# tum-pbs/DMCF

Hardware: AMD Instinct MI355X
Metric: rollout_particle_steps_per_sec (higher is better)
Workload: dtype f32

## Files before the change

dmcf_amd/csrc/cconv_cls.hip:

```cpp

#include "cconv_common.h"

namespace dmcf {

constexpr int kCWaves = 8;
constexpr int kCThreads = 64 * kCWaves;
constexpr int CTM = 2 * kCWaves;
constexpr int kCRows = 16;
constexpr int CCH = 16;
constexpr int kCRow = 1024;
constexpr int kSlots = 96;
constexpr int kHalfSlots = 48;
constexpr int kGrp = 20;
constexpr int kXst = 512;
constexpr int kCMaxNT = 4;
constexpr int kNoPair = 9;

#define CLS_TILE_REGS                                                                                                     \
    "v92", "v93", "v94", "v95", "v96", "v97", "v98", "v99", "v100", "v101", "v102", "v103", "v104", "v105", "v106", "v107", \
        "v108", "v109", "v110", "v111", "v112", "v113", "v114", "v115", "v116", "v117", "v118", "v119", "v120", "v121",    \
        "v122", "v123", "v124", "v125", "v126", "v127"
constexpr int kClsCompilerVgprs = 46;

__device__ __forceinline__ void cls_zero_tiles() {
    asm volatile(
        "v_mov_b32 v92, 0\n\tv_mov_b32 v93, 0\n\tv_mov_b32 v94, 0\n\tv_mov_b32 v95, 0\n\t"
        "v_mov_b32 v96, 0\n\tv_mov_b32 v97, 0\n\tv_mov_b32 v98, 0\n\tv_mov_b32 v99, 0\n\t"
        "v_mov_b32 v100, 0\n\tv_mov_b32 v101, 0\n\tv_mov_b32 v102, 0\n\tv_mov_b32 v103, 0\n\t"
        "v_mov_b32 v104, 0\n\tv_mov_b32 v105, 0\n\tv_mov_b32 v106, 0\n\tv_mov_b32 v107, 0\n\t"
        "v_mov_b32 v108, 0\n\tv_mov_b32 v109, 0\n\tv_mov_b32 v110, 0\n\tv_mov_b32 v111, 0\n\t"
        "v_mov_b32 v112, 0\n\tv_mov_b32 v113, 0\n\tv_mov_b32 v114, 0\n\tv_mov_b32 v115, 0\n\t"
        "v_mov_b32 v116, 0\n\tv_mov_b32 v117, 0\n\tv_mov_b32 v118, 0\n\tv_mov_b32 v119, 0\n\t"
        "v_mov_b32 v120, 0\n\tv_mov_b32 v121, 0\n\tv_mov_b32 v122, 0\n\tv_mov_b32 v123, 0\n\t"
        "v_mov_b32 v124, 0\n\tv_mov_b32 v125, 0\n\tv_mov_b32 v126, 0\n\tv_mov_b32 v127, 0"
        ::: "memory", CLS_TILE_REGS);
}

struct ClsRec {
    float x;
    f32x4 w;
};

__device__ __forceinline__ uint32_t cls_lds_addr(const void* q) {
    return (uint32_t)(uintptr_t)(const __attribute__((address_space(3))) void*)q;
}

__device__ __forceinline__ void xfence() {
    __builtin_amdgcn_fence(__ATOMIC_RELEASE, "wavefront");
    __builtin_amdgcn_wave_barrier();
    __builtin_amdgcn_fence(__ATOMIC_ACQUIRE, "wavefront");
}

template <int NTT, bool NARROW, bool SYM, bool SINGLE, bool PLAIN>
__global__ __launch_bounds__(kCThreads, 4) __attribute__((amdgpu_num_vgpr(kClsCompilerVgprs))) void cconv_cls_kernel(const CconvParams p) {
    extern __shared__ __attribute__((aligned(16))) float smem[];
    const int tid = threadIdx.x, lane = tid & 63;
    const int wave = __builtin_amdgcn_readfirstlane(tid >> 6);
    const int cin = p.cin, cout = p.cout;
    float* Bt = smem;
    float* Gs = smem + CTM * kCRow + wave * kXst;
    unsigned char* Cst = (unsigned char*)(Gs + 24 * kGrp);
    float* Fst = Bt + (wave + kCWaves) * kCRow;
    int* Jst = (int*)(Fst + kHalfSlots * 16);
    const int tile = (int)(blockIdx.x % 8) * p.tiles_per_xcd + (int)(blockIdx.x / 8);
    if (tile >= p.ntiles) return;
    const int64_t pt0 = (int64_t)tile * CTM;
    const int window = PLAIN ? (int)DMCF_WINDOW_POLY6 : p.window;
    const float* const nval = PLAIN ? nullptr : p.nval;
    const float* const imp = PLAIN ? nullptr : p.inp_imp;
    constexpr bool symmetric = SYM;

    const int mk = lane >> 4, mn = lane & 15;
    const float xm = (float)(lane & 3);
    const int widx = (lane >> 2) & 3;
    const int mi = lane & 15, mg = lane >> 4;
    const uint32_t gs_lds = cls_lds_addr(Gs), fst_lds = cls_lds_addr(Fst);
    constexpr uint32_t kOob = 0xffffffffu;
    const uint32_t rowB = (uint32_t)cin * 4u;
    const __amdgpu_buffer_rsrc_t rF = __builtin_amdgcn_make_buffer_rsrc((void*)p.inp_feat, 0, (int)((uint32_t)p.n_inp * rowB), 0x00020000);

    f32x4 acc[NTT];
#pragma unroll
    for (int n = 0; n < NTT; ++n) acc[n] = (f32x4){0.0f, 0.0f, 0.0f, 0.0f};

    float out_prev = 0.0f;
    for (int chunk = 0; chunk < p.nchunks; ++chunk) {
        const int c0 = chunk * CCH;
        const int nch = min(CCH, cin - c0);
        constexpr bool narrow = NARROW;
        const int fr = narrow ? lane >> 1 : lane >> 2, fc4 = narrow ? lane & 1 : lane & 3;
        const int spi = narrow ? 32 : 16;
        const int fstride = narrow ? 8 : 16;
        const bool fch_ok = c0 + 4 * fc4 < cin;
        const int fch = fch_ok ? c0 + 4 * fc4 : 0;
        int64_t rbs[2];
        int nts[2], nbs[2];
        float oxs[2], oys[2], ozs[2];
#pragma unroll
        for (int pp = 0; pp < 2; ++pp) {
            const int64_t i = pt0 + wave + kCWaves * pp;
            rbs[pp] = 0;
            nts[pp] = 0;
            oxs[pp] = oys[pp] = ozs[pp] = 0.0f;
            if (i < p.n_out) {
                const int64_t rb = p.rs[i];
                int64_t re = p.cnt ? rb + p.cnt[i] : p.rs[i + 1];
                if (re > p.pair_cap) re = rb;
                rbs[pp] = rb;
                nts[pp] = (int)min(re - rb, (int64_t)0x7fffffc0);
                oxs[pp] = p.out_pos[3 * i];
                oys[pp] = p.out_pos[3 * i + 1];
                ozs[pp] = p.out_pos[3 * i + 2];
            }
            nbs[pp] = (nts[pp] + 63) >> 6;
        }
        const int nbA = nbs[0], NB = nbs[0] + nbs[1];
        cls_zero_tiles();

        const int nt0 = __builtin_amdgcn_readfirstlane(nts[0]), nt1 = __builtin_amdgcn_readfirstlane(nts[1]);
        const int64_t rb0 = ((int64_t)__builtin_amdgcn_readfirstlane((int)(rbs[0] >> 32)) << 32) | (uint32_t)__builtin_amdgcn_readfirstlane((int)rbs[0]);
        const int64_t rb1 = ((int64_t)__builtin_amdgcn_readfirstlane((int)(rbs[1] >> 32)) << 32) | (uint32_t)__builtin_amdgcn_readfirstlane((int)rbs[1]);
        const int64_t gapB = nt1 > 0 ? rb1 - rb0 : 0;
        const bool near = gapB >= 0 && gapB + nt1 < ((int64_t)1 << 29) && nt0 < (1 << 29);
        const __amdgpu_buffer_rsrc_t rI = __builtin_amdgcn_make_buffer_rsrc(
            (void*)(p.idx + rb0), 0, near ? (int)(max((int64_t)nt0, gapB + nt1) * 4) : 0, 0x00020000);
        const uint32_t offB = (uint32_t)gapB * 4u;
        auto valid = [&](int t) -> bool {
            const bool pp = t >= nbA;
            return t < NB && 64 * (t - (pp ? nbA : 0)) + lane < (pp ? nt1 : nt0);
        };
        auto ld_idx = [&](int t, int& j, float& nv) {
            const bool pp = t >= nbA, ok = valid(t);
            const int o = 64 * (t - (pp ? nbA : 0)) + lane;
            j = 0;
            nv = 0.0f;
            if (near) {
                j = (int)__builtin_amdgcn_raw_buffer_load_b32(rI, ok ? (uint32_t)o * 4u + (pp ? offB : 0u) : kOob, 0, 0);
            } else if (ok) {
                j = p.idx[(pp ? rb1 : rb0) + o];
            }
            if (nval && ok) nv = nval[(pp ? rb1 : rb0) + o];
        };
        auto ld_pos = [&](int j, float& x, float& y, float& z) {
            const float* q = (const float*)((const char*)p.inp_pos + (size_t)__umul24((uint32_t)j, 12u));
            x = q[0];
            y = q[1];
            z = q[2];
        };
        auto geom = [&](int t, int j, float nv, float x, float y, float z, int& cls) -> ClsRec {
            ClsRec c;
            const bool pp = t >= nbA;
            x -= pp ? oxs[1] : oxs[0];
            y -= pp ? oys[1] : oys[0];
            z -= pp ? ozs[1] : ozs[0];
            float a = window_value(window, nval ? nv : rel_dist2(x, y, z), p.inv_r2, p.window_fac);
            if (imp) a *= imp[j];
            filter_coords<false>(x, y, z, p);
            c.x = fminf(3.0f, fmaxf(0.0f, x));
            y = fminf(3.0f, fmaxf(0.0f, y));
            z = fminf(3.0f, fmaxf(0.0f, z));
            const float yf = fminf(floorf(y), 2.0f), zf = fminf(floorf(z), 2.0f);
            const float fy = y - yf, fz = z - zf;
            cls = valid(t) ? 3 * (int)zf + (int)yf : kNoPair;
            const float a0 = a * (1.0f - fz), a1 = a * fz;
            c.w = (f32x4){a0 * (1.0f - fy), a0 * fy, a1 * (1.0f - fy), a1 * fy};
            return c;
        };
        struct Order {
            int pos;
            int cb[10];
        };
        auto order = [&](int cls) -> Order {
            Order o;
            o.pos = 0;
            int base = 0;
#pragma unroll
            for (int c = 0; c < 9; ++c) {
                const uint64_t m = __ballot(cls == c);
                const int rank = __builtin_amdgcn_mbcnt_hi((uint32_t)(m >> 32), __builtin_amdgcn_mbcnt_lo((uint32_t)m, base));
                o.pos = cls == c ? rank : o.pos;
                o.cb[c] = base;
                base += (__builtin_popcountll(m) + 3) & ~3;
            }
            o.cb[9] = base;
            return o;
        };
        auto push_index = [&](int j, int cls, int pos) {
            Jst[lane] = -1;
            if (lane < kSlots - 64) Jst[64 + lane] = -1;
            xfence();
            if (cls != kNoPair) Jst[pos] = (int)__umul24((uint32_t)j, rowB);
        };
        auto push_rec = [&](const ClsRec& c, int cls, int pos) {
            *(f32x4*)(Gs + 4 * lane) = (f32x4){0.0f, 0.0f, 0.0f, 0.0f};
            if (lane < kGrp * 6 - 64) *(f32x4*)(Gs + 4 * (64 + lane)) = (f32x4){0.0f, 0.0f, 0.0f, 0.0f};
            xfence();
            if (cls != kNoPair) {
                float* g = Gs + (pos >> 2) * kGrp + (pos & 3);
                g[16] = c.x;
                *(f32x4*)(g + 3 * (pos & 3)) = c.w;
                if ((pos & 3) == 0) Cst[pos >> 2] = (unsigned char)(4 * cls);
            }
        };
        const uint32_t cbyte = fch_ok ? 4u * (uint32_t)fch : kOob;
        auto f_issue = [&](int h, f32x4 (&f)[3]) {
            uint32_t jo[3];
#pragma unroll
            for (int k = 0; k < 3; ++k) jo[k] = (uint32_t)Jst[kHalfSlots * h + spi * k + fr];
#pragma unroll
            for (int k = 0; k < 3; ++k)
                f[k] = __builtin_bit_cast(f32x4, __builtin_amdgcn_raw_buffer_load_b128(rF, __builtin_elementwise_add_sat(jo[k], cbyte), 0, 0));
        };
        auto f_publish = [&](int t, const f32x4 (&f)[3]) {
            if constexpr (symmetric) {
                f32x4 fi4 = {0.0f, 0.0f, 0.0f, 0.0f};
                if (fch_ok) fi4 = *(const f32x4*)(p.inp_feat + (pt0 + wave + (t >= nbA ? kCWaves : 0)) * cin + fch);
#pragma unroll
                for (int k = 0; k < 3; ++k) *(f32x4*)(Fst + (spi * k + fr) * fstride + 4 * fc4) = f[k] + fi4;
            } else {
#pragma unroll
                for (int k = 0; k < 3; ++k) *(f32x4*)(Fst + (spi * k + fr) * fstride + 4 * fc4) = f[k];
            }
        };
        auto splat = [&](int h, int nslots) {
            const int lo = kHalfSlots * h;
            const int ng = (min(lo + kHalfSlots, nslots) - lo) >> 2;
            const uint32_t pw = gs_lds + ((lo >> 2) * kGrp + 4 * mk + widx) * 4;
            const uint32_t px = gs_lds + ((lo >> 2) * kGrp + 16 + mk) * 4;
            const uint32_t pf = fst_lds + (16 * mk + mn) * 4;
            const uint32_t* cw = (const uint32_t*)(Cst + (lo >> 2));
            const uint32_t c0 = __builtin_amdgcn_readfirstlane(cw[0]), c1 = __builtin_amdgcn_readfirstlane(cw[1]),
                           c2 = __builtin_amdgcn_readfirstlane(cw[2]);
            float xa, wa, fa, xb, wb, fb, av;
            uint32_t sc;
            __builtin_amdgcn_s_setprio(3);
            asm volatile(
#include "cconv_cls_splat.inc"
                : [xa] "=&v"(xa), [wa] "=&v"(wa), [fa] "=&v"(fa), [xb] "=&v"(xb), [wb] "=&v"(wb), [fb] "=&v"(fb),
                  [a] "=&v"(av), [sc] "=&s"(sc)
                : [px] "v"(px), [pw] "v"(pw), [pf] "v"(pf), [xm] "v"(xm), [ng] "s"(ng), [c0] "s"(c0), [c1] "s"(c1), [c2] "s"(c2)
                : "scc", "m0", "memory", CLS_TILE_REGS);
            __builtin_amdgcn_s_setprio(0);
        };
        auto splat8 = [&](int nslots) {
            const int ng = nslots >> 2;
            const uint32_t pw = gs_lds + (4 * mk + widx) * 4;
            const uint32_t px = gs_lds + (16 + mk) * 4;
            const uint32_t pf = fst_lds + (8 * mk + (mn & 7)) * 4;
            const uint32_t* cw = (const uint32_t*)Cst;
            uint32_t c[6];
#pragma unroll
            for (int q = 0; q < 6; ++q) c[q] = __builtin_amdgcn_readfirstlane(cw[q]);
            float xa, wa, fa, xb, wb, fb, av;
            uint32_t sc;
            __builtin_amdgcn_s_setprio(3);
            asm volatile(
#include "cconv_cls_splat8.inc"
                : [xa] "=&v"(xa), [wa] "=&v"(wa), [fa] "=&v"(fa), [xb] "=&v"(xb), [wb] "=&v"(wb), [fb] "=&v"(fb),
                  [a] "=&v"(av), [sc] "=&s"(sc)
                : [px] "v"(px), [pw] "v"(pw), [pf] "v"(pf), [xm] "v"(xm), [ng] "s"(ng), [c0] "s"(c[0]), [c1] "s"(c[1]),
                  [c2] "s"(c[2]), [c3] "s"(c[3]), [c4] "s"(c[4]), [c5] "s"(c[5])
                : "scc", "m0", "memory", CLS_TILE_REGS);
            __builtin_amdgcn_s_setprio(0);
        };
        auto merge = [&](int pt) {
            float* Brow = Bt + pt * kCRow;
            const int gz = lane >> 5, gy = (lane >> 4) & 1;
            const int col = (mn ^ (pt & 15)) << 2;
            const uint32_t mb = cls_lds_addr(Brow + (gz * 4 + gy) * 64 + col);
            xfence();
            asm volatile(
                "s_nop 7\n\ts_nop 7\n\ts_nop 7\n\t"
                "ds_write_b128 %[b], v[92:95] offset:0\n\t"
                "ds_write_b128 %[b], v[100:103] offset:512\n\t"
                "ds_write_b128 %[b], v[116:119] offset:2048\n\t"
                "ds_write_b128 %[b], v[124:127] offset:2560\n\t"
                "ds_read_b128 v[92:95], %[b] offset:256\n\t"
                "s_waitcnt lgkmcnt(0)\n\t"
                "v_add_f32 v92, v92, v96\n\tv_add_f32 v93, v93, v97\n\tv_add_f32 v94, v94, v98\n\tv_add_f32 v95, v95, v99\n\t"
                "ds_write_b128 %[b], v[92:95] offset:256\n\t"
                "ds_read_b128 v[92:95], %[b] offset:2304\n\t"
                "s_waitcnt lgkmcnt(0)\n\t"
                "v_add_f32 v92, v92, v120\n\tv_add_f32 v93, v93, v121\n\tv_add_f32 v94, v94, v122\n\tv_add_f32 v95, v95, v123\n\t"
                "ds_write_b128 %[b], v[92:95] offset:2304\n\t"
                "ds_read_b128 v[92:95], %[b] offset:1024\n\t"
                "s_waitcnt lgkmcnt(0)\n\t"
                "v_add_f32 v92, v92, v104\n\tv_add_f32 v93, v93, v105\n\tv_add_f32 v94, v94, v106\n\tv_add_f32 v95, v95, v107\n\t"
                "ds_write_b128 %[b], v[92:95] offset:1024\n\t"
                "ds_read_b128 v[92:95], %[b] offset:1536\n\t"
                "s_waitcnt lgkmcnt(0)\n\t"
                "v_add_f32 v92, v92, v112\n\tv_add_f32 v93, v93, v113\n\tv_add_f32 v94, v94, v114\n\tv_add_f32 v95, v95, v115\n\t"
                "ds_write_b128 %[b], v[92:95] offset:1536\n\t"
                "ds_read_b128 v[92:95], %[b] offset:1280\n\t"
                "s_waitcnt lgkmcnt(0)\n\t"
                "v_add_f32 v92, v92, v108\n\tv_add_f32 v93, v93, v109\n\tv_add_f32 v94, v94, v110\n\tv_add_f32 v95, v95, v111\n\t"
                "ds_write_b128 %[b], v[92:95] offset:1280\n\t"
                "s_waitcnt lgkmcnt(0)"
                :
                : [b] "v"(mb)
                : "memory", CLS_TILE_REGS);
            cls_zero_tiles();
            xfence();
        };

        if (nbA == 0) merge(wave);
        if (NB > 0) {
            int jA, jB, cl;
            float nvA, nvB, px, py, pz;
            ld_idx(0, jA, nvA);
            ld_idx(1, jB, nvB);
            ld_pos(jA, px, py, pz);
            const ClsRec first = geom(0, jA, nvA, px, py, pz, cl);
            Order oc = order(cl);
            f32x4 ff[3];
            push_index(jA, cl, oc.pos);
            push_rec(first, cl, oc.pos);
            xfence();
            f_issue(0, ff);
            jA = jB;
            nvA = nvB;
            ld_pos(jA, px, py, pz);
            if constexpr (narrow) {
                for (int t = 0; t + 1 < NB; ++t) {
                    const int nslots = oc.cb[9];
                    f_publish(t, ff);
                    ld_idx(t + 2, jB, nvB);
                    const ClsRec nxt = geom(t + 1, jA, nvA, px, py, pz, cl);
                    const Order on = order(cl);
                    push_index(jA, cl, on.pos);
                    jA = jB;
                    nvA = nvB;
                    ld_pos(jA, px, py, pz);
                    xfence();
                    f_issue(0, ff);
                    splat8(nslots);
                    push_rec(nxt, cl, on.pos);
                    oc = on;
                    if (t == nbA - 1) merge(wave);
                }
                f_publish(NB - 1, ff);
                xfence();
                splat8(oc.cb[9]);
                if (NB - 1 == nbA - 1) merge(wave);
            } else {
                for (int t = 0; t + 1 < NB; ++t) {
                    const int nslots = oc.cb[9];
                    const bool two = nslots > kHalfSlots;
                    f_publish(t, ff);
                    ld_idx(t + 2, jB, nvB);
                    if (two) f_issue(1, ff);
                    xfence();
                    splat(0, nslots);
                    const ClsRec nxt = geom(t + 1, jA, nvA, px, py, pz, cl);
                    const Order on = order(cl);
                    push_index(jA, cl, on.pos);
                    xfence();
                    if (two) f_publish(t, ff);
                    jA = jB;
                    nvA = nvB;
                    ld_pos(jA, px, py, pz);
                    f_issue(0, ff);
                    if (two) {
                        xfence();
                        splat(1, nslots);
                    }
                    push_rec(nxt, cl, on.pos);
                    oc = on;
                    if (t == nbA - 1) merge(wave);
                }
                {
                    const int nslots = oc.cb[9];
                    const bool two = nslots > kHalfSlots;
                    f_publish(NB - 1, ff);
                    if (two) f_issue(1, ff);
                    xfence();
                    splat(0, nslots);
                    if (two) {
                        xfence();
                        f_publish(NB - 1, ff);
                        xfence();
                        splat(1, nslots);
                    }
                    if (NB - 1 == nbA - 1) merge(wave);
                }
            }
        }
        if (chunk == p.nchunks - 1) out_prev = epilogue_prefetch(p, pt0, CTM, tid);
        const int nq = (nch + 3) >> 2;
        constexpr int kIt = 64 / kCWaves;
        constexpr int kPre = SINGLE ? (NTT <= 1 ? 8 : (NTT <= 2 ? 4 : 2)) : (NTT <= 1 ? 4 : (NTT <= 2 ? 2 : 1));
        const __amdgpu_buffer_rsrc_t rW = __builtin_amdgcn_make_buffer_rsrc(
            (void*)p.Wp, 0, (int)((uint32_t)p.nchunks * 64u * (uint32_t)p.NT * 1024u), 0x00020000);
        const uint32_t w_lane = ((uint32_t)mg * (uint32_t)p.NT * 16u + (uint32_t)mi) * 16u;
        auto w_issue = [&](int it0, f32x4 (&bw)[kPre][NTT]) {
#pragma unroll
            for (int q = 0; q < kPre; ++q) {
                const int t = wave + kCWaves * (it0 + q);
                if (t < 16 * nq) {
                    int tq, tr;
                    blk_divmod(t, nq, tq, tr);
                    const int blk = tq * 4 + tr;
                    const uint32_t w_blk = (uint32_t)(chunk * 64 + blk) * (uint32_t)p.NT * 1024u;
                    const int wq = 4 * chunk + tr;
                    const uint32_t wm = wq < 8 ? p.wmask >> (4 * wq) : 0xfu;
#pragma unroll
                    for (int n = 0; n < NTT; ++n)
                        if (n < p.NT && ((wm >> n) & 1))
                            bw[q][n] = __builtin_bit_cast(f32x4, __builtin_amdgcn_raw_buffer_load_b128(rW, w_lane, w_blk + 256u * (uint32_t)n, 0));
                }
            }
        };
        f32x4 bw[kPre][NTT];
#pragma unroll
        for (int q = 0; q < kPre; ++q)
#pragma unroll
            for (int n = 0; n < NTT; ++n) asm volatile("" : "=v"(bw[q][n]));
        w_issue(0, bw);
        merge(wave + kCWaves);
        __syncthreads();
        if constexpr (SINGLE) {
#pragma unroll
            for (int n = 0; n < NTT; ++n) acc[n] = (f32x4){0.0f, 0.0f, 0.0f, 0.0f};
        }
#pragma unroll
        for (int it0 = 0; it0 < kIt; it0 += kPre) {
#pragma unroll
            for (int q = 0; q < kPre; ++q) {
                const int t = wave + kCWaves * (it0 + q);
                if (t < 16 * nq) {
                    int tq, tr;
                    blk_divmod(t, nq, tq, tr);
                    const int blk = tq * 4 + tr;
                    const f32x4 av = *(const f32x4*)(Bt + (size_t)mi * kCRow + ((blk * 16 + mg * 4) ^ (mi << 2)));
                    const int wq = 4 * chunk + tr;
                    const uint32_t wm = wq < 8 ? p.wmask >> (4 * wq) : 0xfu;
#pragma unroll
                    for (int n = 0; n < NTT; ++n) {
                        if (n < p.NT && ((wm >> n) & 1)) {
                            const f32x4 bv = bw[q][n];
                            acc[n] = __builtin_amdgcn_mfma_f32_16x16x4f32(av.x, bv.x, acc[n], 0, 0, 0);
                            acc[n] = __builtin_amdgcn_mfma_f32_16x16x4f32(av.y, bv.y, acc[n], 0, 0, 0);
                            acc[n] = __builtin_amdgcn_mfma_f32_16x16x4f32(av.z, bv.z, acc[n], 0, 0, 0);
                            acc[n] = __builtin_amdgcn_mfma_f32_16x16x4f32(av.w, bv.w, acc[n], 0, 0, 0);
                        }
                    }
                }
            }
            if (it0 + kPre < kIt && wave + kCWaves * (it0 + kPre) < 16 * nq) w_issue(it0 + kPre, bw);
        }
        __syncthreads();
    }

    float* red = Bt;
    const int ncol = 16 * p.NT;
#pragma unroll
    for (int n = 0; n < NTT; ++n) {
        if (n < p.NT) {
#pragma unroll
            for (int r = 0; r < 4; ++r) red[((size_t)wave * kCRows + 4 * mg + r) * ncol + n * 16 + mi] = acc[n][r];
        }
    }
    __syncthreads();
    for (int e = tid; e < CTM * cout; e += kCThreads) {
        const int ptt = e / cout, o = e % cout;
        const int64_t ii = pt0 + ptt;
        if (ii >= p.n_out) continue;
        float v = 0.0f;
#pragma unroll
        for (int w = 0; w < kCWaves; ++w) v += red[((size_t)w * kCRows + ptt) * ncol + o];
        if (p.bias) v += p.bias[o];
        float* dst = p.out + ii * cout + o;
        if (p.flags & DMCF_FLAG_ACCUMULATE) v += e == tid ? out_prev : *dst;
        *dst = v;
    }
}

static constexpr size_t kClsLds = (size_t)(CTM * kCRow + kCWaves * kXst) * sizeof(float);

size_t cconv_cls_packed_floats(int cin, int cout) {
    const int nchunks = (cin + CCH - 1) / CCH, NT = (cout + 15) / 16;
    return (size_t)nchunks * 64 * 4 * NT * 16 * 4 + 16;
}

__global__ void pack_filter_cls(const float* __restrict__ src, float* __restrict__ dst, int cin, int cout, int nchunks, int NT,
                                int symmetric, int sym_axis) {
    const int64_t total = (int64_t)nchunks * 64 * 4 * NT * 16 * 4 + 16;
    const int hd[3] = {(symmetric && sym_axis == 0) ? 2 : 4, (symmetric && sym_axis == 1) ? 2 : 4,
                       (symmetric && sym_axis == 2) ? 2 : 4};
    for (int64_t e = (int64_t)blockIdx.x * blockDim.x + threadIdx.x; e < total; e += (int64_t)gridDim.x * blockDim.x) {
        int64_t s = e;
        const int q = (int)(s & 3); s >>= 2;
        const int j = (int)(s & 15); s >>= 4;
        const int n = (int)(s % NT); s /= NT;
        const int g = (int)(s & 3); s >>= 2;
        const int blk = (int)(s & 63); s >>= 6;
        const int chunk = (int)s;
        const int ci = chunk * CCH + 4 * (blk & 3) + g, o = 16 * n + j;
        float v = 0.0f;
        if (chunk < nchunks && ci < cin && o < cout) {
            int c3[3] = {blk >> 4, (blk >> 2) & 3, q};
            float sign = 1.0f;
            if (symmetric) {
                const int hh = hd[sym_axis];
                if (c3[sym_axis] >= hh) {
                    c3[sym_axis] -= hh;
                } else {
                    sign = -1.0f;
                    for (int a = 0; a < 3; ++a) c3[a] = hd[a] - 1 - c3[a];
                }
            }
            v = sign * src[((((int64_t)c3[0] * hd[1] + c3[1]) * hd[2] + c3[2]) * cin + ci) * cout + o];
        }
        dst[e] = v;
    }
}

static bool cls_eligible(const dmcf_cconv_args* a, int dz, int dy, int dx, bool forced) {
    if (!cconv_fast444(a, dz, dy, dx) || !cconv_offsets_fit_24bit(a)) return false;
    if (a->filter_dims[4] > 16 * kCMaxNT) return false;
    if (forced) return true;
    return a->filter_dims[3] >= 8;
}

size_t cconv_cls_workspace_floats(const dmcf_cconv_args* a, int, int, int, bool) {
    return cconv_cls_packed_floats(a->filter_dims[3], a->filter_dims[4]);
}

bool cconv_cls_prepare(CconvParams& p, const dmcf_cconv_args* a, int tm, void* workspace, hipStream_t stream) {
    float* packed = (float*)workspace;
    p.NT = (p.cout + 15) / 16;
    p.nchunks = (p.cin + CCH - 1) / CCH;
    const int64_t total = (int64_t)cconv_cls_packed_floats(p.cin, p.cout);
    const unsigned g = (unsigned)((total + 255) / 256);
    if (!(a->flags & DMCF_FLAG_FILTER_PACKED))
        hipLaunchKernelGGL(pack_filter_cls, dim3(g < 2048u ? g : 2048u), dim3(256), 0, stream, a->filters, packed, p.cin, p.cout,
                           p.nchunks, p.NT, (a->flags & DMCF_FLAG_SYMMETRIC) ? 1 : 0, a->sym_axis);
    p.Wp = packed;
    return cconv_set_tiles(p, tm);
}

static void cls_pick(const dmcf_cconv_args* a, int, int, int, CconvPick& k) {
    const int cin = a->filter_dims[3], NT = (a->filter_dims[4] + 15) / 16;
    const bool sym = (a->flags & DMCF_FLAG_SYMMETRIC) != 0;
    const bool plain = !sym && cconv_plain(a);
#define CLS_PICK(NARROW, SINGLE)                                                                \
    (sym ? CCONV_KERNEL_NT(NT, cconv_cls_kernel, NARROW, true, SINGLE, false)                   \
         : (plain ? CCONV_KERNEL_NT(NT, cconv_cls_kernel, NARROW, false, SINGLE, true)          \
                  : CCONV_KERNEL_NT(NT, cconv_cls_kernel, NARROW, false, SINGLE, false)))
    const CconvKernel f = cin <= 8 ? CLS_PICK(true, true) : (cin <= CCH ? CLS_PICK(false, true) : CLS_PICK(false, false));
#undef CLS_PICK
    k = {f.fn, f.name, kClsLds, kCThreads, cconv_cls_packed_floats(cin, a->filter_dims[4])};
}

static int cls_launch(CconvParams p, const dmcf_cconv_args* a, int, int, int, const CconvPick& k, void* workspace, hipStream_t stream) {
    if (!cconv_cls_prepare(p, a, CTM, workspace, stream)) return DMCF_EUNSUPPORTED;
    void* kargs[] = {(void*)&p};
    return cconv_launch_kernel(k, dim3((unsigned)p.tiles_per_xcd * 8u), kargs, stream);
}

CconvForm cconv_cls_form = {'c', cls_eligible, cls_pick, cconv_cls_workspace_floats, cls_launch};

}
```

dmcf_amd/models/pbf_model.py:

```python
import os

import numpy as np
import torch

from .. import ops
from ..utils import convolutions as _convs
from ..utils.convolutions import ContinuousConv, PointSampling
from ..utils.tools.losses import (get_loss, compute_density, compute_pressure, compute_transformed_dx, get_dilated_pos,
                                  get_window_func)
from .base_model import BaseModel, Dense


def align_vector(v0, v1):
    v0n = v0 / (torch.linalg.norm(v0) + 1e-9)
    v1n = v1 / (torch.linalg.norm(v1) + 1e-9)
    v = torch.linalg.cross(v0n, v1n)
    c = torch.dot(v0n, v1n)
    s = torch.linalg.norm(v)
    if float(s) < 1e-6:
        return torch.eye(3, device=v0.device) * (-1.0 if float(c) < 0 else 1.0)
    zero = torch.zeros((), device=v0.device)
    vx = torch.stack([torch.stack([zero, -v[2], v[1]]), torch.stack([v[2], zero, -v[0]]),
                      torch.stack([-v[1], v[0], zero])])
    return torch.eye(3, device=v0.device) + vx + (vx @ vx) / (1 + c)


class PBFNet(BaseModel):
    def __init__(self, name="PBFNet", kernel_size=[4, 4, 4], channels=16, strides=[1], particle_radii=[0.05],
                 coordinate_mapping="ball_to_cube_volume_preserving", interpolation="linear", window=None,
                 window_dens=None, ignore_query_points=False, grav=-9.81, transformation={}, loss=None,
                 timestep=0.01, dens_radius=None, circular=False, dens_feats=False, pres_feats=False, equivar=False,
                 use_vel=True, use_acc=True, use_feats=False, use_box_feats=True, use_pre_adv=False, use_bnds=True,
                 dens_norm=False, rest_dens=3.5, stiffness=20.0, voxel_size=None, centralize=False,
                 out_scale=[0.01, 0.01, 0.01], sample_pad=0, sample_hyst=0.1, part_scale=1.0, **kwargs):
        super().__init__(name=name, **kwargs)
        if dens_radius is None:
            dens_radius = particle_radii
        self.equivar = equivar
        self.kernel_size = kernel_size
        self.channel = channels
        self.strides = strides
        self.particle_radii = particle_radii
        self.coordinate_mapping = coordinate_mapping
        self.interpolation = interpolation
        self.window = window
        self.ignore_query_points = ignore_query_points
        self.voxel_size = None if voxel_size is None else np.asarray(voxel_size, dtype=np.float32)
        self.centralize = centralize
        self.circular = circular
        self.transformation = transformation or {}
        self.sample_pad = sample_pad
        self.sample_hyst = sample_hyst
        self.dens_radius = dens_radius
        self.dens_feats = dens_feats
        self.pres_feats = pres_feats
        self.dens_norm = dens_norm
        self.rest_dens = rest_dens
        self.stiffness = stiffness
        self.out_scale = [float(v) for v in out_scale]
        self.window_dens = window_dens
        self.use_vel = use_vel
        self.use_acc = use_acc
        self.use_feats = use_feats
        self.use_box_feats = use_box_feats
        self.use_pre_adv = use_pre_adv
        self.use_bnds = use_bnds
        self.timestep = timestep
        self.grav = grav
        self.part_scale = part_scale
        self.num_fluid_neighbors = 1
        self.loss_fn = {}
        for l, v in (loss or {}).items():
            v = dict(v)
            if v.get("typ") == "dense" and "radius" not in v:
                v["radius"] = dens_radius[0]
            self.loss_fn[l] = get_loss(**v)

        self._all_convs = []
        self.fluid_convs = self.get_cconv(name="fluid_obs", filters=channels, activation=None,
                                          window_func=self.window, circular=circular)
        self.fluid_dense = Dense(units=channels, name="fluid_dense")
        self.obs_convs = self.get_cconv(name="obs_conv", filters=channels, activation=None,
                                        window_func=self.window, circular=circular)
        self.obs_dense = Dense(units=channels, name="obs_dense")
        if dens_norm:
            self.sampling = PointSampling(name="sampling", window_function=get_window_func(window_dens), normalize=True)
        if self.equivar:
            self.scale_dens = Dense(units=1, name="scale")
            self.rot_dens = Dense(units=4, name="rot")
        if self.use_pre_adv:
            self.adv_convs = torch.nn.ModuleList([
                self.get_cconv(name="adv_conv0", filters=channels, activation=None, window_func=self.window,
                               circular=circular),
                self.get_cconv(name="adv_conv1", filters=channels, activation=None, window_func=self.window,
                               circular=circular)])
            self.adv_dense = torch.nn.ModuleList([Dense(units=channels, name="adv_dense0"),
                                                  Dense(units=channels, name="adv_dense1")])
        self.setup()

    def setup(self):
        return

    @property
    def num_fluid_neighbors(self):
        if self._num_fluid_neighbors is None and getattr(self, "_fluid_counts", None) is not None:
            self._num_fluid_neighbors, self._fluid_counts = self._fluid_counts(), None
        return self._num_fluid_neighbors

    @num_fluid_neighbors.setter
    def num_fluid_neighbors(self, value):
        self._num_fluid_neighbors = value
        self._fluid_counts = None

    def get_cconv(self, name, kernel_size=None, activation=None, ignore_query_points=None, window_func=None,
                  normalize=False, **kwargs):
        if kernel_size is None:
            kernel_size = self.kernel_size
        if ignore_query_points is None:
            ignore_query_points = self.ignore_query_points
        conv = ContinuousConv(name=name, kernel_size=kernel_size, activation=activation, align_corners=True,
                              interpolation=self.interpolation, coordinate_mapping=self.coordinate_mapping,
                              normalize=normalize, window_function=get_window_func(window_func),
                              radius_search_ignore_query_points=ignore_query_points,
                              use_dense_layer_for_center=False, **kwargs)
        self._all_convs.append((name, conv))
        return conv

    conv_hook = None
    ghost_prefetch = None
    shard = None

    def apply_conv(self, conv, feats, inp_pos, out_pos, extent, widest_extent=None):
        if self.conv_hook is not None:
            return self.conv_hook(conv, feats, inp_pos, out_pos, extent, widest_extent)
        return conv(feats, inp_pos, out_pos, extent, None)

    def integrate_pos_vel(self, pos1, vel1, acc1=None):
        dt = self.timestep
        if acc1 is None:
            acc1 = ops.const_tensor([0.0, self.grav, 0.0], torch.float32, pos1.device)
        vel2 = vel1 + dt * acc1
        pos2 = pos1 + dt * vel2
        return pos2, vel2

    def compute_new_pos_vel(self, pos1, vel1, pos2, vel2, pos_correction):
        dt = self.timestep
        pos = pos2 + pos_correction
        vel = (pos - pos1) / dt
        return pos, vel

    def transform(self, data, training=True, **kwargs):
        pos, vel, acc, feats, box, bfeats = data
        dev = pos.device
        if "translate" in self.transformation:
            translate = ops.const_tensor(self.transformation["translate"], torch.float32, dev)
            pos = pos + translate
            box = box + translate
        if "scale" in self.transformation:
            scale = ops.const_tensor(self.transformation["scale"], torch.float32, dev)
            pos = pos * scale
            box = box * scale
            vel = vel * scale
            if acc is not None:
                acc = acc * scale
        if "grav_eqvar" in self.transformation:
            grav_eqvar = ops.const_tensor(self.transformation["grav_eqvar"], torch.float32, dev)
            self.R = align_vector(grav_eqvar, acc[0])
            pos, vel, acc, box, bfeats = (x @ self.R for x in (pos, vel, acc, box, bfeats))
        return [pos, vel, acc, feats, box, bfeats]

    def inv_transform(self, prev, data, **kwargs):
        pos, vel = prev
        dev = pos.device
        if "grav_eqvar" in self.transformation:
            R = self.R.t()
            pos = pos @ R
            vel = vel @ R
        if "scale" in self.transformation:
            scale = ops.const_tensor([max(float(v), 1e-5) for v in self.transformation["scale"]], torch.float32, dev)
            pos = pos / scale
            vel = vel / scale
        if "translate" in self.transformation:
            pos = pos - ops.const_tensor(self.transformation["translate"], torch.float32, dev)
        return pos, vel

    def preprocess(self, data, training=True, vel_corr=None, tape=None, **kwargs):
        _pos, _vel, acc, feats, box, bfeats = data
        if vel_corr is not None:
            vel = vel_corr
            pos = _pos + vel * self.timestep
        else:
            pos, vel = self.integrate_pos_vel(_pos, _vel, acc)
        filter_extent = [float(np.float32(r) * np.float32(2)) for r in self.particle_radii]
        if not pos.shape[0]:
            mn, mx = pos.new_full((3,), 3.0e38), pos.new_full((3,), -3.0e38)
        elif pos.is_cuda:
            mn, mx = ops.points_aabb(pos)
        else:
            mn, mx = torch.aminmax(pos.t().contiguous(), dim=1)
        if self.shard is not None:
            mn, mx = self.shard.fluid_bounds(mn, mx)
        lo = mn - filter_extent[-1]
        hi = mx + filter_extent[-1]
        fltr = ((box >= lo) & (box <= hi)).all(dim=1)
        keep = fltr.nonzero().flatten()
        box = box.index_select(0, keep)
        bfeats = bfeats.index_select(0, keep)

        fluid_feats = [torch.ones_like(pos[:, :1])]
        if self.use_vel:
            fluid_feats.append(vel)
        if self.use_acc:
            if acc is None:
                raise ValueError("use_acc=True needs per-particle accelerations (pbf_model.py:341-342)")
            fluid_feats.append(acc)
        if self.use_feats:
            fluid_feats.append(feats)
        box_feats = [torch.ones_like(box[:, :1])]
        if self.use_box_feats:
            box_feats.append(bfeats)
        all_pos = torch.cat([pos, box], dim=0)
        self.all_pos = all_pos
        if self.shard is not None:
            self.shard.begin(all_pos, pos, box)
        dens = None
        if self.dens_feats or self.dens_norm or self.pres_feats:
            win = get_window_func(self.window_dens)
            dens = compute_density(all_pos, all_pos, self.dens_radius[0], win=win)
            n_fluid = pos.shape[0]
            if self.dens_feats:
                fluid_feats.append(dens[:n_fluid].unsqueeze(-1))
                box_feats.append(dens[n_fluid:].unsqueeze(-1))
            if self.pres_feats:
                pres = compute_pressure(all_pos, all_pos, dens, self.rest_dens, win=win, stiffness=self.stiffness)
                fluid_feats.append(pres[:n_fluid].unsqueeze(-1))
                box_feats.append(pres[n_fluid:].unsqueeze(-1))
        fluid_feats = torch.cat(fluid_feats, dim=-1)
        box_feats = torch.cat(box_feats, dim=-1)
        self.inp_feats = fluid_feats
        self.inp_bfeats = box_feats

        fused = self._fused_input_convs(fluid_feats, box_feats, pos, all_pos, filter_extent[0])
        if fused is not None:
            ans_conv, ans_obs = fused
        else:
            ans_conv = self.apply_conv(self.fluid_convs, fluid_feats * self.part_scale, pos, all_pos, filter_extent[0])
            ans_obs = self.apply_conv(self.obs_convs, box_feats * self.part_scale, box, all_pos, filter_extent[0])
        ans_dense = self.fluid_dense(fluid_feats)
        ans_dense_obs = self.obs_dense(box_feats)
        ans_dense = torch.cat([ans_dense, ans_dense_obs], dim=0)
        if self.use_pre_adv:
            _all_pos = torch.cat([_pos, box], dim=0)
            pre_adv_feats = torch.ones_like(_pos[:, :1])
            if self.use_vel:
                pre_adv_feats = torch.cat([pre_adv_feats, _vel], dim=-1)
            ans_adv = self.adv_convs[0](pre_adv_feats * self.part_scale, _pos, all_pos, filter_extent[0], None)
            ans_dens_adv = torch.cat([self.adv_dense[0](pre_adv_feats), ans_dense_obs], dim=0)
            fluid_feats = torch.cat([ans_conv, ans_obs, ans_adv, ans_dense, ans_dens_adv], dim=-1)
        else:
            fluid_feats = torch.cat([ans_conv, ans_obs, ans_dense], dim=-1)

        if self.shard is not None:
            dilated_pos, idx = self.shard.dilated_pos(all_pos if self.use_bnds else pos)
        else:
            dilated_pos, _, idx = get_dilated_pos(all_pos if self.use_bnds else pos, self.strides,
                                                  voxel_size=self.voxel_size, centralize=self.centralize,
                                                  pad=self.sample_pad, hyst=self.sample_hyst)
        if self.dens_norm:
            dens = [(dens if self.use_bnds else dens[:pos.shape[0]]).unsqueeze(-1)]
            for scale in range(1, len(self.dens_radius)):
                d = self.sampling(dens[-1], dilated_pos[scale - 1], dilated_pos[scale], self.dens_radius[scale], None)
                dens.append(torch.clamp(d, min=1e-2))
        else:
            dens = None
        self.dilated_pos = dilated_pos
        return [dilated_pos, fluid_feats, idx, dens]

    def fused_input_operands(self, fluid_feats, box_feats):
        a, b = self.fluid_convs, self.obs_convs
        if (os.environ.get("DMCF_FUSE_INPUT_CONVS", "1") == "0" or _convs._CACHE.depth == 0 or not fluid_feats.is_cuda
                or self.recording()):
            return None
        if ops.search_set() != "distance":
            return None
        wa, wb = a.window_function, b.window_function
        if a.kernel is None or b.kernel is None:
            return None
        same = (isinstance(wa, _convs.WindowFunction) and isinstance(wb, _convs.WindowFunction) and wa.name == wb.name
                and wa.fac == wb.fac and tuple(a.kernel.shape[:3]) == tuple(b.kernel.shape[:3]) and a.filters == b.filters
                and all(getattr(a, k) == getattr(b, k) for k in (
                    "align_corners", "coordinate_mapping", "interpolation", "normalize", "use_bias",
                    "radius_search_ignore_query_points", "radius_search_metric", "use_dense_layer_for_center"))
                and not (a.symmetric or b.symmetric or a.circular or b.circular or a.normalize
                         or a.radius_search_ignore_query_points or a.use_dense_layer_for_center)
                and a.activation is None and b.activation is None
                and a.kernel.shape[3] == fluid_feats.shape[1] and b.kernel.shape[3] == box_feats.shape[1])
        if not same:
            return None
        n, m, cf, cb, co = fluid_feats.shape[0], box_feats.shape[0], fluid_feats.shape[1], box_feats.shape[1], a.filters
        cin = -(-(cf + cb) // 4) * 4
        feats = fluid_feats.new_zeros((n + m, cin))
        feats[:n, :cf] = fluid_feats * self.part_scale
        feats[n:, cf:cf + cb] = box_feats * self.part_scale
        kernel = a.kernel.new_zeros(tuple(a.kernel.shape[:3]) + (cin, 2 * co))
        kernel[..., :cf, :co] = a.kernel
        kernel[..., cf:cf + cb, co:] = b.kernel
        bias = torch.cat([a.bias, b.bias]) if a.use_bias else None
        return feats, kernel, bias

    def fused_input_conv(self, kernel, bias, feats, inp_pos, out_pos, extent):
        a = self.fluid_convs
        radius = float(np.float32(0.5) * np.float32(extent))
        nns = _convs._CACHE.search(a.fixed_radius_search, inp_pos, out_pos, radius, distances=False)
        index, row_splits, raw_dist = nns.raw()
        out = ops.cconv_forward(kernel, out_pos, extent, inp_pos, feats, index, row_splits, neighbors_value=raw_dist,
                                window=a.window_function.name, window_fac=a.window_function.fac,
                                align_corners=a.align_corners, coordinate_mapping=a.coordinate_mapping,
                                interpolation=a.interpolation, bias=bias, n_pairs_ref=_convs.pairs_ref(nns),
                                neighbors_row_count=getattr(nns, "row_count", None))
        a.nns = self.obs_convs.nns = None
        return out, nns

    def _fused_input_convs(self, fluid_feats, box_feats, pos, all_pos, extent):
        operands = self.fused_input_operands(fluid_feats, box_feats)
        if operands is None:
            return None
        feats, kernel, bias = operands
        n, co = fluid_feats.shape[0], self.fluid_convs.filters
        if self.conv_hook is not None:
            out = self.apply_conv(lambda f, pi, po, ext, _: self.fused_input_conv(kernel, bias, f, pi, po, ext)[0],
                                  feats, all_pos, all_pos, extent)
            self._fluid_counts = None
            return out[:, :co].contiguous(), out[:, co:].contiguous()
        out, nns = self.fused_input_conv(kernel, bias, feats, all_pos, all_pos, extent)
        index = nns.raw()[0]
        row_count = getattr(nns, "row_count", None)
        if row_count is not None:
            stride = nns.stride

            def count():
                rows = index[:n * stride].view(n, stride)
                cols = torch.arange(stride, device=index.device, dtype=torch.int32)
                return ((rows < n) & (cols[None, :] < row_count[:n, None])).sum(dim=1).to(torch.float32)
        else:
            idx, rs = nns.neighbors_index, nns.neighbors_row_splits

            def count():
                return ops.reduce_subarrays_sum((idx < n).to(torch.float32), rs)[:n]
        self._fluid_counts = count
        return out[:, :co].contiguous(), out[:, co:].contiguous()

    def loss_keys(self):
        return self.loss_fn.keys()

    def loss(self, results, data):
        pred, target = results[0], data[1]
        return {n: l(target, pred, num_fluid_neighbors=self.num_fluid_neighbors, input=data[0], target_prev=data[2],
                     pre_steps=data[3], pos_correction=self.pos_correction)
                for n, l in self.loss_fn.items()}

    def postprocess(self, prev, data, training=True, vel_corr=None, **kwargs):
        pos, vel, acc = data[:3]
        pcnt = pos.shape[0]
        if self.shard is not None:
            self._num_fluid_neighbors = None
        elif self.fluid_convs.nns is None and getattr(self, "_fluid_counts", None) is not None:
            self._num_fluid_neighbors = None
        else:
            counts = ops.neighbor_counts(self.fluid_convs.nns)
            self.num_fluid_neighbors = counts[:pcnt]

        out = prev
        if self.equivar:
            if self.shard is not None:
                raise NotImplementedError("equivar in a sharded step (its search has no ghost plan)")
            scale = self.scale_dens(out)
            if scale.shape[0] != self.all_pos.shape[0]:
                raise NotImplementedError("equivar with use_bnds=False: the scale has %d rows for %d points (the reference's own "
                                          "gather is out of range there)" % (scale.shape[0], self.all_pos.shape[0]))
            out = compute_transformed_dx(self.all_pos, scale, None, radius=self.particle_radii[0])
        if out.shape[-1] == 1:
            out = out.repeat(1, 3)
        elif out.shape[-1] == 2:
            out = torch.cat([out, out[:, :1]], dim=-1)
        out_scale = ops.const_tensor(self.out_scale, torch.float32, pos.device)
        self.net_output = out
        self.pos_correction = out_scale * out[:pcnt]
        self.obs = out_scale * out[pcnt:]
        if vel_corr is not None:
            vel2 = vel_corr
            pos2 = pos + vel2 * self.timestep
        else:
            pos2, vel2 = self.integrate_pos_vel(pos, vel, acc)
        pos2_corrected, vel2_corrected = self.compute_new_pos_vel(pos, vel, pos2, vel2, self.pos_correction)
        return [pos2_corrected, vel2_corrected]
```

Before: 13.37 million.

## Add joint single-pass classification path for short neighbor rows in cls cconv

```diff
diff --git a/dmcf_amd/csrc/cconv_cls.hip b/dmcf_amd/csrc/cconv_cls.hip
--- a/dmcf_amd/csrc/cconv_cls.hip
+++ b/dmcf_amd/csrc/cconv_cls.hip
@@ -15,6 +15,7 @@
 constexpr int kXst = 512;
 constexpr int kCMaxNT = 4;
 constexpr int kNoPair = 9;
+constexpr int kJointSlots = 128;
 
 #define CLS_TILE_REGS                                                                                                     \
     "v92", "v93", "v94", "v95", "v96", "v97", "v98", "v99", "v100", "v101", "v102", "v103", "v104", "v105", "v106", "v107", \
@@ -51,7 +52,7 @@
     __builtin_amdgcn_fence(__ATOMIC_ACQUIRE, "wavefront");
 }
 
-template <int NTT, bool NARROW, bool SYM, bool SINGLE, bool PLAIN>
+template <int NTT, bool NARROW, bool SYM, bool SINGLE, bool PLAIN, bool JOINT = false>
 __global__ __launch_bounds__(kCThreads, 4) __attribute__((amdgpu_num_vgpr(kClsCompilerVgprs))) void cconv_cls_kernel(const CconvParams p) {
     extern __shared__ __attribute__((aligned(16))) float smem[];
     const int tid = threadIdx.x, lane = tid & 63;
@@ -147,12 +148,8 @@
             y = q[1];
             z = q[2];
         };
-        auto geom = [&](int t, int j, float nv, float x, float y, float z, int& cls) -> ClsRec {
+        auto geom_rel = [&](bool ok, int j, float nv, float x, float y, float z, int& cls) -> ClsRec {
             ClsRec c;
-            const bool pp = t >= nbA;
-            x -= pp ? oxs[1] : oxs[0];
-            y -= pp ? oys[1] : oys[0];
-            z -= pp ? ozs[1] : ozs[0];
             float a = window_value(window, nval ? nv : rel_dist2(x, y, z), p.inv_r2, p.window_fac);
             if (imp) a *= imp[j];
             filter_coords<false>(x, y, z, p);
@@ -161,10 +158,17 @@
             z = fminf(3.0f, fmaxf(0.0f, z));
             const float yf = fminf(floorf(y), 2.0f), zf = fminf(floorf(z), 2.0f);
             const float fy = y - yf, fz = z - zf;
-            cls = valid(t) ? 3 * (int)zf + (int)yf : kNoPair;
+            cls = ok ? 3 * (int)zf + (int)yf : kNoPair;
             const float a0 = a * (1.0f - fz), a1 = a * fz;
             c.w = (f32x4){a0 * (1.0f - fy), a0 * fy, a1 * (1.0f - fy), a1 * fy};
             return c;
+        };
+        auto geom = [&](int t, int j, float nv, float x, float y, float z, int& cls) -> ClsRec {
+            const bool pp = t >= nbA;
+            x -= pp ? oxs[1] : oxs[0];
+            y -= pp ? oys[1] : oys[0];
+            z -= pp ? ozs[1] : ozs[0];
+            return geom_rel(valid(t), j, nv, x, y, z, cls);
         };
         struct Order {
             int pos;
@@ -303,6 +307,135 @@
             xfence();
         };
 
+        bool joint = false;
+        if constexpr (JOINT) {
+            joint = nt0 <= 64 && nt1 <= 64 && nt0 + nt1 <= 64 && nt0 + nt1 > 0;
+        if (joint) {
+            constexpr int kGH = narrow ? 24 : 12;
+            float* Xs = Fst + kHalfSlots * 16 + kJointSlots;
+            const uint32_t xs_lds = cls_lds_addr(Xs);
+            const bool pB = lane >= nt0, ok = lane < nt0 + nt1;
+            const int o = pB ? lane - nt0 : lane;
+            int j = 0, cl;
+            float nv = 0.0f, qx, qy, qz;
+            if (near) {
+                j = (int)__builtin_amdgcn_raw_buffer_load_b32(rI, ok ? (uint32_t)o * 4u + (pB ? offB : 0u) : kOob, 0, 0);
+            } else if (ok) {
+                j = p.idx[(pB ? rb1 : rb0) + o];
+            }
+            if (nval && ok) nv = nval[(pB ? rb1 : rb0) + o];
+            ld_pos(j, qx, qy, qz);
+            qx -= pB ? oxs[1] : oxs[0];
+            qy -= pB ? oys[1] : oys[0];
+            qz -= pB ? ozs[1] : ozs[0];
+            const ClsRec rec = geom_rel(ok, j, nv, qx, qy, qz, cl);
+            const int cl18 = ok ? cl + (pB ? 9 : 0) : 18;
+            int pos = 0, S = 0, SA = 0;
+#pragma unroll
+            for (int c = 0; c < 18; ++c) {
+                if (c == 9) SA = S;
+                const uint64_t m = __ballot(cl18 == c);
+                const int rank = __builtin_amdgcn_mbcnt_hi((uint32_t)(m >> 32), __builtin_amdgcn_mbcnt_lo((uint32_t)m, S));
+                pos = cl18 == c ? rank : pos;
+                S += (__builtin_popcountll(m) + 3) & ~3;
+            }
+            S = __builtin_amdgcn_readfirstlane(S);
+            SA = __builtin_amdgcn_readfirstlane(SA);
+            Jst[lane] = -1;
+            Jst[64 + lane] = -1;
+            *(f32x4*)(Gs + 4 * lane) = (f32x4){0.0f, 0.0f, 0.0f, 0.0f};
+            if (lane < kGrp * 6 - 64) *(f32x4*)(Gs + 4 * (64 + lane)) = (f32x4){0.0f, 0.0f, 0.0f, 0.0f};
+            if (lane < kGrp * 5 / 4) *(f32x4*)(Xs + 4 * lane) = (f32x4){0.0f, 0.0f, 0.0f, 0.0f};
+            xfence();
+            if (ok) {
+                Jst[pos] = (int)__umul24((uint32_t)j, rowB);
+                const int gi = pos >> 2;
+                float* g = (gi < 24 ? Gs + gi * kGrp : Xs + (gi - 24) * kGrp) + (pos & 3);
+                g[16] = rec.x;
+                *(f32x4*)(g + 3 * (pos & 3)) = rec.w;
+                if ((pos & 3) == 0) Cst[gi] = (unsigned char)(4 * cl);
+            }
+            xfence();
+            auto f_issue_j = [&](int h, f32x4 (&f)[3]) {
+                uint32_t jo[3];
+#pragma unroll
+                for (int k = 0; k < 3; ++k) {
+                    const int s = 4 * kGH * h + spi * k + fr;
+                    jo[k] = s < kJointSlots ? (uint32_t)Jst[s] : kOob;
+                }
+#pragma unroll
+                for (int k = 0; k < 3; ++k)
+                    f[k] = __builtin_bit_cast(f32x4, __builtin_amdgcn_raw_buffer_load_b128(rF, __builtin_elementwise_add_sat(jo[k], cbyte), 0, 0));
+            };
+            auto f_publish_j = [&](int h, const f32x4 (&f)[3]) {
+                if constexpr (symmetric) {
+                    f32x4 fiA = {0.0f, 0.0f, 0.0f, 0.0f}, fiB = {0.0f, 0.0f, 0.0f, 0.0f};
+                    if (fch_ok && nt0 > 0) fiA = *(const f32x4*)(p.inp_feat + (pt0 + wave) * cin + fch);
+                    if (fch_ok && nt1 > 0) fiB = *(const f32x4*)(p.inp_feat + (pt0 + wave + kCWaves) * cin + fch);
+#pragma unroll
+                    for (int k = 0; k < 3; ++k)
+                        *(f32x4*)(Fst + (spi * k + fr) * fstride + 4 * fc4) = f[k] + (4 * kGH * h + spi * k + fr < SA ? fiA : fiB);
+                } else {
+#pragma unroll
+                    for (int k = 0; k < 3; ++k) *(f32x4*)(Fst + (spi * k + fr) * fstride + 4 * fc4) = f[k];
+                }
+            };
+            auto splat_j = [&](int g0, int ng, int gh) {
+                const uint32_t rb = g0 < 24 ? gs_lds + (uint32_t)(g0 * kGrp * 4) : xs_lds + (uint32_t)((g0 - 24) * kGrp * 4);
+                const uint32_t pw = rb + (4 * mk + widx) * 4;
+                const uint32_t px = rb + (16 + mk) * 4;
+                const uint32_t pf = fst_lds + ((g0 - gh) * 4 * fstride + (narrow ? 8 * mk + (mn & 7) : 16 * mk + mn)) * 4;
+                constexpr int NW = narrow ? 6 : 3;
+                const uint32_t* cw = (const uint32_t*)Cst + (g0 >> 2);
+                const int sh = 8 * (g0 & 3);
+                uint32_t w[NW + 1], c[NW];
+#pragma unroll
+                for (int q = 0; q <= NW; ++q) w[q] = __builtin_amdgcn_readfirstlane(cw[q]);
+#pragma unroll
+                for (int q = 0; q < NW; ++q) c[q] = (uint32_t)(((((uint64_t)w[q + 1]) << 32) | w[q]) >> sh);
+                ng = __builtin_amdgcn_readfirstlane(ng);
+                float xa, wa, fa, xb, wb, fb, av;
+                uint32_t sc;
+                __builtin_amdgcn_s_setprio(3);
+                if constexpr (narrow) {
+                    asm volatile(
+#include "cconv_cls_splat8.inc"
+                        : [xa] "=&v"(xa), [wa] "=&v"(wa), [fa] "=&v"(fa), [xb] "=&v"(xb), [wb] "=&v"(wb), [fb] "=&v"(fb),
+                          [a] "=&v"(av), [sc] "=&s"(sc)
+                        : [px] "v"(px), [pw] "v"(pw), [pf] "v"(pf), [xm] "v"(xm), [ng] "s"(ng), [c0] "s"(c[0]), [c1] "s"(c[1]),
+                          [c2] "s"(c[2]), [c3] "s"(c[NW - 3]), [c4] "s"(c[NW - 2]), [c5] "s"(c[NW - 1])
+                        : "scc", "m0", "memory", CLS_TILE_REGS);
+                } else {
+                    asm volatile(
+#include "cconv_cls_splat.inc"
+                        : [xa] "=&v"(xa), [wa] "=&v"(wa), [fa] "=&v"(fa), [xb] "=&v"(xb), [wb] "=&v"(wb), [fb] "=&v"(fb),
+                          [a] "=&v"(av), [sc] "=&s"(sc)
+                        : [px] "v"(px), [pw] "v"(pw), [pf] "v"(pf), [xm] "v"(xm), [ng] "s"(ng), [c0] "s"(c[0]), [c1] "s"(c[1]), [c2] "s"(c[2])
+                        : "scc", "m0", "memory", CLS_TILE_REGS);
+                }
+                __builtin_amdgcn_s_setprio(0);
+            };
+            const int NG = S >> 2, gb = SA >> 2;
+            f32x4 ff[3];
+            f_issue_j(0, ff);
+            bool mergedA = false;
+            for (int G0 = 0; G0 < NG; G0 += kGH) {
+                const int G1 = min(G0 + kGH, NG);
+                if (G0 > 0) xfence();
+                f_publish_j(G0 / kGH, ff);
+                if (G1 < NG) f_issue_j(G0 / kGH + 1, ff);
+                xfence();
+                const int ga = min(max(gb, G0), G1);
+                if (ga > G0) splat_j(G0, ga - G0, G0);
+                if (!mergedA && gb <= G1) {
+                    merge(wave);
+                    mergedA = true;
+                }
+                if (G1 > ga) splat_j(ga, G1 - ga, G0);
+            }
+        }
+        }
+        if (!joint) {
         if (nbA == 0) merge(wave);
         if (NB > 0) {
             int jA, jB, cl;
@@ -385,6 +518,7 @@
                 }
             }
         }
+        }
         if (chunk == p.nchunks - 1) out_prev = epilogue_prefetch(p, pt0, CTM, tid);
         const int nq = (nch + 3) >> 2;
         constexpr int kIt = 64 / kCWaves;
@@ -539,6 +673,11 @@
     return cconv_set_tiles(p, tm);
 }
 
+static int cls_joint_env() {
+    const char* e = getenv("DMCF_CLS_JOINT");
+    return e ? (e[0] == '0' ? 0 : 1) : -1;
+}
+
 static void cls_pick(const dmcf_cconv_args* a, int, int, int, CconvPick& k) {
     const int cin = a->filter_dims[3], NT = (a->filter_dims[4] + 15) / 16;
     const bool sym = (a->flags & DMCF_FLAG_SYMMETRIC) != 0;
@@ -547,8 +686,19 @@
     (sym ? CCONV_KERNEL_NT(NT, cconv_cls_kernel, NARROW, true, SINGLE, false)                   \
          : (plain ? CCONV_KERNEL_NT(NT, cconv_cls_kernel, NARROW, false, SINGLE, true)          \
                   : CCONV_KERNEL_NT(NT, cconv_cls_kernel, NARROW, false, SINGLE, false)))
-    const CconvKernel f = cin <= 8 ? CLS_PICK(true, true) : (cin <= CCH ? CLS_PICK(false, true) : CLS_PICK(false, false));
+    CconvKernel f = cin <= 8 ? CLS_PICK(true, true) : (cin <= CCH ? CLS_PICK(false, true) : CLS_PICK(false, false));
 #undef CLS_PICK
+    const int jenv = cls_joint_env();
+    if (cin <= CCH && (jenv < 0 ? (a->row_length_hint == 1 && cin <= 8) : jenv == 1)) {
+#define CLS_JOINT(...) CconvKernel{(const void*)cconv_cls_kernel<__VA_ARGS__, true>, "cconv_cls_kernel<" #__VA_ARGS__ ">"}
+#define CLS_JOINT_NT(...) (NT <= 1 ? CLS_JOINT(1, __VA_ARGS__) : (NT <= 2 ? CLS_JOINT(2, __VA_ARGS__) : CLS_JOINT(4, __VA_ARGS__)))
+#define CLS_PICK_J(NARROW) \
+    (sym ? CLS_JOINT_NT(NARROW, true, true, false) : (plain ? CLS_JOINT_NT(NARROW, false, true, true) : CLS_JOINT_NT(NARROW, false, true, false)))
+        f = cin <= 8 ? CLS_PICK_J(true) : CLS_PICK_J(false);
+#undef CLS_PICK_J
+#undef CLS_JOINT_NT
+#undef CLS_JOINT
+    }
     k = {f.fn, f.name, kClsLds, kCThreads, cconv_cls_packed_floats(cin, a->filter_dims[4])};
 }
 
diff --git a/dmcf_amd/models/pbf_model.py b/dmcf_amd/models/pbf_model.py
--- a/dmcf_amd/models/pbf_model.py
+++ b/dmcf_amd/models/pbf_model.py
@@ -317,7 +317,8 @@
                                 window=a.window_function.name, window_fac=a.window_function.fac,
                                 align_corners=a.align_corners, coordinate_mapping=a.coordinate_mapping,
                                 interpolation=a.interpolation, bias=bias, n_pairs_ref=_convs.pairs_ref(nns),
-                                neighbors_row_count=getattr(nns, "row_count", None))
+                                neighbors_row_count=getattr(nns, "row_count", None),
+                                row_length_hint=1)
         a.nns = self.obs_convs.nns = None
         return out, nns
 
```

Result: no change. 13.30 million (-0.5%).
